# garfieldnate/ray_tracer_challenge

Measured on AMD Instinct MI355X. Metric: Mrays/s, higher is better.
Workload: dtype f32

## Files before the change

ray_tracer_challenge_amd/_lib.py:

```python
import ctypes as C
import os

HERE = os.path.dirname(os.path.abspath(__file__))
LIB_PATH = os.environ.get("RTC_AMD_LIB") or os.path.join(HERE, "librtc_amd.so")

RTC_OK = 0
RTC_ERR_INVALID_ARG, RTC_ERR_UNSUPPORTED, RTC_ERR_NO_LIGHT, RTC_ERR_DEVICE, RTC_ERR_NO_DEVICE = -1, -2, -3, -4, -5
RTC_SPHERE, RTC_PLANE, RTC_CUBE, RTC_CYLINDER, RTC_CONE, RTC_TRIANGLE = 0, 1, 2, 3, 4, 5
(RTC_PATTERN_NONE, RTC_PATTERN_STRIPES, RTC_PATTERN_GRADIENT, RTC_PATTERN_RINGS, RTC_PATTERN_CHECKERS,
 RTC_PATTERN_SINE2D, RTC_PATTERN_TEXTURE_MAP, RTC_PATTERN_CUBE_MAP) = 0, 1, 2, 3, 4, 5, 6, 7
RTC_UV_CHECKERS, RTC_UV_ALIGN_CHECK, RTC_UV_IMAGE = 1, 2, 3
RTC_MAP_SPHERICAL, RTC_MAP_PLANAR, RTC_MAP_CYLINDRICAL = 1, 2, 3
RTC_LIGHT_POINT, RTC_LIGHT_RECT = 0, 1
RTC_JITTER_CONSTANT, RTC_JITTER_HASHED, RTC_JITTER_SEQUENCE = 0, 2, 3
RTC_MAX_DEPTH = 255
RTC_STACK_DEPTH_BASE = 8

FP = C.POINTER(C.c_float)


class rtc_uv_pattern(C.Structure):
    _fields_ = [("kind", C.c_int32), ("width", C.c_float), ("height", C.c_float), ("colors", (C.c_float * 3) * 5),
                ("image_width", C.c_uint32), ("image_height", C.c_uint32), ("image_rgb", C.POINTER(C.c_float))]

# ... 184 lines not shown
         "rtc_diag_refine_block_list": (C.c_uint32, [C.POINTER(C.c_uint32), C.POINTER(C.c_uint32), C.c_uint32, C.c_uint32, C.c_uint32, C.c_double,
                                                     C.c_double, C.c_double, C.POINTER(C.c_uint32), C.c_uint32]),
         "rtc_diag_simulate_dispatch": (C.c_double, [C.POINTER(C.c_uint32), C.c_uint32, C.c_uint32]),
         "rtc_diag_band_walk": (C.c_uint32, [C.c_uint32, C.c_uint32, C.POINTER(rtc_partition), C.POINTER(C.c_uint32), C.c_uint32, C.POINTER(C.c_uint64)]),
         "rtc_diag_scene_tiles": (C.c_uint64, [C.POINTER(C.c_uint8), C.c_uint32, C.c_uint32, C.c_uint32, C.c_uint32, C.POINTER(rtc_partition),
                                               C.POINTER(C.c_uint32), C.POINTER(C.c_uint32), C.c_uint32, C.POINTER(C.c_uint32)]),
         "rtc_diag_rect_launch": (C.c_uint64, [C.c_uint32, C.c_uint32, C.POINTER(rtc_partition), C.POINTER(C.c_uint32), C.c_uint32, C.c_int32,
                                               C.c_uint32, C.POINTER(C.c_uint32)]),
         "rtc_diag_ss_plan": (C.c_uint32, [C.c_uint32, C.c_uint32, C.POINTER(C.c_uint32), C.POINTER(C.c_uint32), C.c_uint32, C.c_uint32, C.c_uint32,
                                           C.c_double, C.POINTER(C.c_uint32), C.c_uint32, C.POINTER(C.c_uint32)]),
         "rtc_diag_ctx_share_log2": (C.c_uint32, [C.c_void_p]),
         "rtc_diag_adaptive_plan": (C.c_uint32, [C.c_uint32, C.c_uint32, C.c_uint32, C.c_uint32, C.c_uint32, C.c_uint64, C.c_uint32,
                                                 C.POINTER(C.c_uint32), C.POINTER(C.c_uint32)]),
         "rtc_diag_ray_keys": (None, [FP, FP, C.c_uint32, FP, C.POINTER(C.c_uint32)]),
         "rtc_diag_reorder_plan": (C.c_uint32, [C.c_uint32, C.c_uint32, C.POINTER(C.c_uint32)]),
         "rtc_diag_scene_plan": (C.c_int, [C.POINTER(rtc_scene), C.POINTER(rtc_camera), C.c_char_p, C.c_uint32, C.POINTER(C.c_uint64)])}

_lib = None
_loaded = {}
DEV_LIB_PATH = os.path.join(HERE, "librtc_amd_dev.so")


class RtcError(RuntimeError):
    def __init__(self, status, message):
        super().__init__("rtc status %d: %s" % (status, message))
        self.status = status


def _preload_torch_hip_runtime():
    import importlib.util
    import sys
# ... 11 lines not shown
            C.CDLL(path, mode=C.RTLD_GLOBAL)
        except OSError:
            pass


def load(path):
    path = os.path.abspath(path)
    if path not in _loaded:
        if not os.path.exists(path):
            raise ImportError(
                "%s is missing: build it with `python -m ray_tracer_challenge_amd.build%s` "
                "(there is no CPU/Python fallback for the render path)" % (path, " --dev" if path.endswith("_dev.so") else ""))
        _preload_torch_hip_runtime()
        L = C.CDLL(path)
        for name, (res, args) in list(SIGNATURES.items()) + list(EXTRA.items()):
            fn = getattr(L, name)
            fn.restype = res
            fn.argtypes = args
        _loaded[path] = L
    return _loaded[path]


def lib():
    global _lib
    if _lib is None:
        _lib = load(LIB_PATH)
    return _lib


class use_library:

# ... 22 lines not shown
```

ray_tracer_challenge_amd/api.py:

```python
import ctypes as C

import numpy as np

from . import _lib as L

f32 = np.float32


def _a(x, n=None):
    arr = np.ascontiguousarray(np.asarray(x, dtype=f32).reshape(-1))
    if n is not None and arr.size != n:
        raise ValueError("expected %d values, got %d" % (n, arr.size))
    return arr


_FLOAT_ARRAYS = {}


def _p(arr):
    n = arr.size
    t = _FLOAT_ARRAYS.get(n)
    if t is None:
        t = _FLOAT_ARRAYS[n] = C.c_float * n
    try:
# ... 690 lines not shown
        self.light = light

    def _c(self):
        return _CScene(self)

    def validate(self, camera=None):
        cs = self._c()
        L.check(L.lib().rtc_scene_validate(C.byref(cs.scene), C.byref(camera._cam) if camera is not None else None))

    def scene_plan(self, camera=None):
        cs = self._c()
        text, digests = C.create_string_buffer(1 << 16), (C.c_uint64 * 4)()
        L.check(L.lib().rtc_diag_scene_plan(C.byref(cs.scene), C.byref(camera._cam) if camera is not None else None, text, len(text), digests))
        return tuple(digests), dict(line.split("=", 1) for line in text.value.decode().splitlines())

    def color_at(self, origins, directions, depth, device=0):
        o = np.ascontiguousarray(np.asarray(origins, dtype=f32).reshape(-1, 4))
        d = np.ascontiguousarray(np.asarray(directions, dtype=f32).reshape(-1, 4))
        out = np.zeros((o.shape[0], 3), dtype=f32)
        cs = self._c()
        L.check(L.lib().rtc_color_at(C.byref(cs.scene), _p(o), _p(d), o.shape[0], int(depth), device, _p(out)))
        return out

    def hit_at(self, origins, directions, light=True, device=0, planes=None):
        o = np.ascontiguousarray(np.asarray(origins, dtype=f32).reshape(-1, 4))
        d = np.ascontiguousarray(np.asarray(directions, dtype=f32).reshape(-1, 4))
        names = list(L.HIT_PLANES) if planes is None else list(planes)
        if not light:
            names = [k for k in names if k != "light"]
        n = o.shape[0]
# ... 190 lines not shown
```

ray_tracer_challenge_amd/csrc/rtc_device.hip:

```cpp
#include <hip/hip_runtime.h>
#include <hip/hiprtc.h>

#include <dlfcn.h>
#include <sys/stat.h>
#include <unistd.h>

#include <cerrno>
#include <chrono>

#include <algorithm>
#include <array>
#include <functional>
#include <queue>
#include <cmath>
#include <cstdio>
#include <cstdlib>
#include <cstring>
#include <fstream>
#include <map>
#include <mutex>
#include <sstream>
#include <string>
#include <utility>
#include <set>
// ... 96 lines not shown
    std::vector<std::string> spec_defs;
    std::string spec_name;
    typedef std::map<int, std::pair<hipFunction_t, std::string>> DeepKernels;
    DeepKernels deep_fn;
    std::string kernel_name;
    int tree_waves = 6;
    bool lazy_jit = false;
    bool jit_deferred = false;
    std::vector<uint8_t> heavy_tiles;
    uint32_t heavy_w = 0, heavy_h = 0;
    std::map<std::array<uint32_t, 5>, BlockList> block_lists;
    float scene_box_coverage = 1.0f;
    uint32_t scene_rect[4] = {0u, 0u, 0u, 0u};
    std::vector<uint8_t> scene_tile_mask;
    uint32_t scene_tiles_w = 0u, scene_tiles_h = 0u;
    struct SceneTileList {
        uint32_t* d = nullptr;
        size_t n = 0;
        unsigned long long traced_pixels = 0ull;
        uint2* d_fill = nullptr;
        size_t n_fill = 0;
    };
    hipStream_t fill_stream = nullptr;
    hipEvent_t ev_fork = nullptr, ev_join = nullptr;
    std::map<std::array<uint32_t, 3>, SceneTileList> scene_tile_lists;
    float scene_rect_coverage = 1.0f;
    std::string kernel_id;
    std::string jit_note;
    std::vector<float4> soa_host;
    std::set<std::pair<const void*, const void*>> warmed;
    std::vector<float> texels_host;
    uint4* d_block_counts = nullptr;
    size_t block_cap = 0;
    void* h_feedback = nullptr;
    size_t h_feedback_cap = 0;
    WfRay* d_wf_rays[4] = {nullptr, nullptr, nullptr, nullptr};
// ... 86 lines not shown
            }
            if (recut) {
                bl.scene_changes = 0u;
                bl.best_ms = bl.loss_ms = 0.0;
                bl.state = timed ? BlockList::TIMED : BlockList::FRESH;
                bl.passes = c->policy.feedback_passes ? c->policy.feedback_passes - 1u : 0u;
            }
        }
        ++it;
    }
}
static void drop_scene_tile_lists(rtc_ctx* c) {
    for (auto& tl : c->scene_tile_lists) {
        if (tl.second.d) (void)hipFree(tl.second.d);
        if (tl.second.d_fill) (void)hipFree(tl.second.d_fill);
    }
    c->scene_tile_lists.clear();
}
static void drop_block_lists(rtc_ctx* c) {
    for (auto& bl : c->block_lists) {
        if (bl.second.d) (void)hipFree(bl.second.d);
        if (bl.second.d_ticks) (void)hipFree(bl.second.d_ticks);
        if (bl.second.ev0) (void)hipEventDestroy(bl.second.ev0);
        if (bl.second.ev1) (void)hipEventDestroy(bl.second.ev1);
    }
    c->block_lists.clear();
}

namespace {

// ... 397 lines not shown
}

static rtc_status order_grid(rtc_ctx* c, BlockList& bl, uint32_t gx, uint32_t gy, uint32_t rows) {
    const Policy& P = c->policy;
    HIP_TRY(hipDeviceSynchronize());
    const size_t nt = bl.n;
    std::vector<uint32_t> launched(nt), ordered;
    void* staging = nullptr;
    HIP_TRY(feedback_staging(c, 4u * nt * sizeof(uint4), &staging));
    uint32_t* ticks = (uint32_t*)staging;
    if (bl.counts) {
        const uint4* counts = (const uint4*)staging;
        HIP_TRY(hipMemcpy(staging, bl.d_ticks, 4u * nt * sizeof(uint4), hipMemcpyDeviceToHost));
        for (size_t i = 0; i < 4u * nt; i++) {
            const uint4 n = counts[i];
            ticks[i] = (n.x - std::min(n.x, n.z)) + 16u * n.y + n.z / 8u;
        }
    } else {
        HIP_TRY(hipMemcpy(staging, bl.d_ticks, 4u * nt * sizeof(uint32_t), hipMemcpyDeviceToHost));
    }
    for (uint32_t by = 0; by < gy; by++)
        for (uint32_t bx = 0; bx < gx; bx++) {
            uint32_t x = bx, y = by;
            if (bl.swizzled) {
                const uint32_t j = (by & 3u) * gx + bx, r = j & 7u;
                y = (by & ~3u) + (r >> 1);
                x = 2u * (j >> 3) + (r & 1u);
            }
            launched[(size_t)by * gx + bx] = tile_word(0u, 16u * x, 16u * y);
        }
    const double wave_slots = 0.85 * 4.0 * compute_units(c) * 6.0;
    bl.state = BlockList::REFINED;
    bl.listed = false;
    {
        std::vector<uint32_t> block_cost(nt), sorted_cost;
        for (size_t b = 0; b < nt; b++) block_cost[b] = std::max(std::max(ticks[4 * b], ticks[4 * b + 1]), std::max(ticks[4 * b + 2], ticks[4 * b + 3]));
        sorted_cost = block_cost;
        std::sort(sorted_cost.begin(), sorted_cost.end(), std::greater<uint32_t>());
        const size_t wg_slots = (size_t)(wave_slots / 4.0);
        const double in_order = simulate_dispatch(block_cost, wg_slots), longest_first = simulate_dispatch(sorted_cost, wg_slots);
        if (P.jit_print) std::fprintf(stderr, "librtc_amd: grid of %zu blocks: modelled frame %.4g in image order, %.4g longest first\n", nt, in_order, longest_first);
        if (!(longest_first < 0.97 * in_order)) return RTC_OK;
    }
    refine_block_list(launched, ticks, c->hdr.width, rows, wave_slots, INFINITY, 0.0, &ordered);
    if (ordered.empty() || ordered.size() > bl.n) return RTC_OK;
    HIP_TRY(grow(&bl.d, &bl.d_cap, ordered.size(), true));
    std::memcpy(staging, ordered.data(), ordered.size() * sizeof(uint32_t));
    HIP_TRY(hipMemcpy(bl.d, staging, ordered.size() * sizeof(uint32_t), hipMemcpyHostToDevice));
    bl.n_listed = ordered.size();
    bl.listed = true;
    return RTC_OK;
}

static hipError_t launch_render(rtc_ctx* c, hipFunction_t spec_fn, dim3 grid, hipStream_t stream, RenderArgs& a) {
    if (c->ss_k != 1u) {
        SsRenderArgs sa;
        sa.fine = a;
// ... 96 lines not shown
    if (!resident) {
        c->soa_host.swap(soa);
        c->texels_host.swap(texels);
    }
    if (same_frame && P.block_feedback) restart_block_lists(c);
    else drop_block_lists(c);
    drop_scene_tile_lists(c);
    c->deep_fn.clear();
    c->simple = plan.simple;
    c->heavy_tiles.swap(plan.heavy_tiles), c->heavy_w = plan.heavy_w, c->heavy_h = plan.heavy_h;
    c->scene_box_coverage = plan.scene_box_coverage;
    std::memcpy(c->scene_rect, plan.scene_rect, sizeof(c->scene_rect));
    c->scene_rect_coverage = plan.scene_rect_coverage;
    c->scene_tile_mask.swap(plan.scene_tile_mask);
    if (!c->scene_tile_mask.empty()) c->scene_tiles_w = plan.scene_tiles_w, c->scene_tiles_h = plan.scene_tiles_h;
    c->spec_shares = plan.spec_shares, c->spec_blocks_y = plan.spec_blocks_y, c->spec_rect = plan.spec_rect;
    if (plan.tree_waves) c->tree_waves = plan.tree_waves;
    c->wf_pays = plan.wf_pays;
    c->wf_disabled = false;
    c->kernel_name = plan.family_name;
    c->spec_defs = plan.spec_defs;
    c->spec_name = plan.spec_name;
    {
        rtc_ctx::Trace& t = c->trace;
        t.defs.clear();
        for (const auto& d : plan.spec_defs)
            t.defs.push_back((d == "-DRTC_SPEC_BLOCKS_Y=1" || d == "-DRTC_SPEC_RECT=1" || d == "-DRTC_SPEC_SHARE=1") ? d.substr(0, d.size() - 1) + "0" : d);
        if (!t.defs.empty()) t.defs.push_back("-DRTC_SPEC_TRACE=1");
        auto renamed = [](const std::string& name) { return name.rfind("render_", 0) == 0 ? "trace_" + name.substr(7) : name; };
        t.family_name = renamed(plan.family_name), t.spec_name = renamed(plan.spec_name);
// ... 158 lines not shown
        c->wf_disabled = true;
        c->events_used--;
        return RTC_OK;
    }
    c->rendered = true;
    c->wf_last = true;
    *used = true;
    return RTC_OK;
}

struct LaunchLists {
    const uint32_t* d_tiles = nullptr;
    uint32_t* d_ticks = nullptr;
    BlockList* timed_list = nullptr;
    void* copy_counts_to = nullptr;
    const rtc_ctx::SceneTileList* scene_tiles = nullptr;
};

static bool scene_recurses(const rtc_ctx* c) {
    const uint32_t stride = padded_count(c->hdr.n_objects);
    for (uint32_t i = 0; i < c->hdr.n_objects; i++) {
        const float4 mb = c->soa_host[soa_index(COL_MAT_B, stride, i)], mc = c->soa_host[soa_index(COL_MAT_C, stride, i)];
        if (!(mb.w == 0.0f) || !(mc.x == 0.0f)) return true;
    }
    return false;
}

static rtc_status block_list_room(rtc_ctx* c) {
    if (c->block_lists.size() >= 256u) {
        HIP_TRY(hipDeviceSynchronize());
        drop_block_lists(c);
// ... 32 lines not shown
        if (bl.state == BlockList::FRESH) {
            bl.state = BlockList::TIMED;
        } else {
            if (bl.ev0 == nullptr) {
                HIP_TRY(hipEventCreate(&bl.ev0));
                HIP_TRY(hipEventCreate(&bl.ev1));
            }
            L->timed_list = &bl;
        }
    }
    L->d_tiles = bl.d;
    lp->run_list(bl.n);
    return RTC_OK;
}

static rtc_status use_scene_tile_list(rtc_ctx* c, const Partition& q, hipStream_t stream, const rtc_ctx::SceneTileList** out) {
    const std::array<uint32_t, 3> key = {q.band_rows, q.n_parts, q.part};
    auto it = c->scene_tile_lists.find(key);
    if (it == c->scene_tile_lists.end()) {
        SceneTilePlan host;
        plan_scene_tiles(TileMask{c->scene_tile_mask.data(), c->scene_tiles_w, c->scene_tiles_h}, c->hdr.width, c->hdr.height, q, &host);
        static_assert(sizeof(FillRun) == sizeof(uint2), "fill_tiles_kernel reads the runs as uint2");
        rtc_ctx::SceneTileList tl;
        tl.n = host.tiles.size();
        tl.n_fill = host.fill.size();
        tl.traced_pixels = host.traced_pixels;
        if (tl.n) {
            HIP_TRY(hipMalloc((void**)&tl.d, tl.n * sizeof(uint32_t)));
            HIP_TRY(hipMemcpyAsync(tl.d, host.tiles.data(), tl.n * sizeof(uint32_t), hipMemcpyHostToDevice, stream));
            if (tl.n_fill) {
                HIP_TRY(hipMalloc((void**)&tl.d_fill, tl.n_fill * sizeof(uint2)));
                HIP_TRY(hipMemcpyAsync(tl.d_fill, host.fill.data(), tl.n_fill * sizeof(uint2), hipMemcpyHostToDevice, stream));
            }
            HIP_TRY(hipStreamSynchronize(stream));
        }
        it = c->scene_tile_lists.emplace(key, tl).first;
    }
    if (it->second.n && !c->fill_stream) {
        HIP_TRY(hipStreamCreateWithFlags(&c->fill_stream, hipStreamNonBlocking));
        HIP_TRY(hipEventCreateWithFlags(&c->ev_fork, hipEventDisableTiming));
        HIP_TRY(hipEventCreateWithFlags(&c->ev_join, hipEventDisableTiming));
    }
    *out = &it->second;
    return RTC_OK;
}

static rtc_status use_grid_feedback(rtc_ctx* c, const Partition& q, uint32_t rows, int32_t depth, bool timed_waves, hipStream_t stream, LaunchPlan* lp,
                                    LaunchLists* L) {
    const std::array<uint32_t, 5> key = {q.band_rows, q.n_parts, q.part, 0xffffffffu, (uint32_t)depth};
    auto it = c->block_lists.find(key);
    if (it == c->block_lists.end()) {
        RTC_TRY(block_list_room(c));
        BlockList bl;
        bl.n = lp->n_workgroups();
        bl.state = BlockList::IDLE;
        it = c->block_lists.emplace(key, bl).first;
    }
    BlockList& bl = it->second;
// ... 61 lines not shown
    a.block_x0 = lp.block_x0, a.block_y0 = lp.block_y0;
    a.fill_wg_rows = lp.fill_wg_rows, a.fill_rows = lp.fill_rows, a.fill_period = lp.fill_period;
    a.fill_x0 = lp.fill_rect[0], a.fill_x1 = lp.fill_rect[1], a.fill_y0 = lp.fill_rect[2], a.fill_y1 = lp.fill_rect[3];
    return a;
}

static bool wavefront_wanted(const rtc_ctx* c, uint32_t rows, int32_t depth) {
    return c->hdr.n_trav != 0u && rows > 0u && depth >= 1 && depth <= RTC_STACK_DEPTH_BASE && (int)depth < (int)WF_MAX_LEVELS && !c->wf_disabled &&
           (size_t)rows * c->hdr.width <= (16u << 20) && c->policy.wavefront == 1 && c->ss_k == 1u;
}

static rtc_status settle_shape(rtc_ctx* c, const Partition& q, uint32_t rows, int32_t depth, uint32_t share_log2, hipFunction_t spec_fn, void* d_out_rgb,
                               bool out_u8, const ProgressPlan* progress, hipStream_t stream, LaunchPlan* lp, LaunchLists* L) {
    const Policy& P = c->policy;
    const bool list_words_fit = c->hdr.width <= 65532u && rows <= 131068u;
    if (lp->shape == LaunchPlan::GRID && share_log2 == 0u && !c->scene_tile_mask.empty() && (q.band_rows & 15u) == 0u && list_words_fit) {
        RTC_TRY(use_scene_tile_list(c, q, stream, &L->scene_tiles));
        if (L->scene_tiles->n) {
            lp->run_scene_tiles(L->scene_tiles->n, c->last_pixels - L->scene_tiles->traced_pixels);
            L->d_tiles = L->scene_tiles->d;
        }
    }
    if (lp->shape == LaunchPlan::GRID && share_log2 == 0u && c->scene_rect[0] < c->scene_rect[1] && c->scene_rect_coverage < P.scene_rect_threshold() &&
        (spec_fn == nullptr || c->spec_rect)) {
        plan_rect_launch(lp, c->hdr.width, c->hdr.height, q, rows, c->last_pixels, c->scene_rect, P.blocks_y == 0 ? 1u : lp->blocks_y, out_u8, P.fill_wgs);
        if (out_u8) HIP_TRY(hipMemsetAsync(d_out_rgb, 0, (size_t)rows * c->hdr.width * 3u, stream));
    }
    if (P.swizzle && lp->plain_grid()) lp->pad_for_swizzle();
    if (lp->plain_grid() && P.block_feedback && P.grid_feedback && progress == nullptr && share_log2 == 0u && list_words_fit &&
        !(c->hdr.n_trav != 0u && P.wavefront))
        RTC_TRY(use_grid_feedback(c, q, rows, depth, spec_fn && c->spec_shares, stream, lp, L));
    if (progress && progress->d_done && lp->plain_grid()) plan_chunks(lp, progress->want_chunks, PROGRESS_MAX_CHUNKS);
// ... 129 lines not shown
        if (n < cap) bands[3 * n] = y0, bands[3 * n + 1] = y1, bands[3 * n + 2] = local0;
        n++;
        for (uint32_t y = y0; y < y1; y++) inverts = inverts && global_row(q, local0 + (y - y0)) == y;
    });
    facts[0] = partition_rows(height, part), facts[1] = traced_pixels(width, height, q), facts[2] = inverts ? 1u : 0u;
    return n;
}
uint64_t rtc_diag_scene_tiles(const uint8_t* mask, uint32_t mask_w, uint32_t mask_h, uint32_t width, uint32_t height, const rtc_partition* part,
                              uint32_t* tiles, uint32_t* fill , uint32_t cap, uint32_t counts[2]) {
    SceneTilePlan plan;
    plan_scene_tiles(TileMask{mask, mask_w, mask_h}, width, height, resolve(part), &plan);
    for (size_t i = 0; i < plan.tiles.size() && i < cap; i++) tiles[i] = plan.tiles[i];
    for (size_t i = 0; i < plan.fill.size() && i < cap; i++) fill[2 * i] = plan.fill[i].x0_n, fill[2 * i + 1] = plan.fill[i].row;
    counts[0] = (uint32_t)plan.tiles.size(), counts[1] = (uint32_t)plan.fill.size();
    return plan.traced_pixels;
}
uint64_t rtc_diag_rect_launch(uint32_t width, uint32_t height, const rtc_partition* part, const uint32_t rect[4], uint32_t blocks_y, int32_t out_u8,
                              uint32_t fill_wgs, uint32_t out[12]) {
    const Partition q = resolve(part);
    LaunchPlan lp;
    plan_rect_launch(&lp, width, height, q, partition_rows(height, part), traced_pixels(width, height, q), rect, blocks_y, out_u8 != 0, fill_wgs);
    const uint32_t v[12] = {lp.grid_x, lp.grid_y, lp.blocks_y, lp.block_x0, lp.block_y0, lp.fill_wg_rows, lp.fill_rows, lp.fill_period,
                            lp.fill_rect[0], lp.fill_rect[1], lp.fill_rect[2], lp.fill_rect[3]};
    std::memcpy(out, v, sizeof(v));
    return lp.extra_rays;
}

uint32_t rtc_diag_ctx_share_log2(rtc_ctx* c) { return c ? c->last_share_log2 : 0u; }
uint32_t rtc_diag_ss_plan(uint32_t k, uint32_t share_log2, const uint32_t* list, const uint32_t* ticks, uint32_t n, uint32_t width, uint32_t rows,
                          double wave_slots, uint32_t* out, uint32_t cap, uint32_t* n_out) {
// ... 1026 lines not shown
```

ray_tracer_challenge_amd/csrc/rtc_launch_plan.h:

```cpp
#ifndef RTC_LAUNCH_PLAN_H
#define RTC_LAUNCH_PLAN_H

#include <algorithm>
#include <cstdint>
#include <cstring>
#include <functional>
#include <queue>
#include <vector>

#include "rtc_internal.h"

namespace rtc {

struct TileMask {
    const uint8_t* bits;
    uint32_t w, h;
};

inline uint32_t tile_word(uint32_t s, uint32_t x0, uint32_t y0) { return (s & 3u) << 30 | (x0 / 4u) << 16 | (s >> 2) << 15 | (y0 / 4u); }
inline uint32_t tile_s(uint32_t t) { return (t >> 30) | ((t >> 13) & 4u); }
inline uint32_t tile_x0(uint32_t t) { return ((t >> 16) & 0x3fffu) << 2; }
inline uint32_t tile_y0(uint32_t t) { return (t & 0x7fffu) << 2; }
inline uint32_t ss_max_share_log2(uint32_t k) { return k == 4u ? 2u : 4u; }
constexpr uint32_t ADAPTIVE_STEP_SLOTS = 64u;
// ... 147 lines not shown
                if (!mask.bits[(size_t)ty * mask.w + tx]) {
                    if (run == 0u) run0 = tx;
                    run++;
                    continue;
                }
                close_run();
                out->tiles.push_back(tile_word(0u, tx * 16u, yl));
                const uint32_t px1 = std::min(width - 1u, tx * 16u + 16u), py1 = std::min(std::min(height - 1u, y1), ty * 16u + 16u);
                if (px1 > tx * 16u && py1 > ty * 16u) out->traced_pixels += (unsigned long long)(px1 - tx * 16u) * (py1 - ty * 16u);
            }
            close_run();
        }
    });
}

struct LaunchPlan {
    enum Shape { GRID, BLOCK_LIST, SCENE_TILES, SCENE_RECT } shape = GRID;
    uint32_t grid_x = 0u, grid_y = 0u;
    uint32_t block_h = 16u;
    uint32_t blocks_y = 1u;
    uint32_t block_x0 = 0u, block_y0 = 0u;
    bool swizzle = false;
    uint32_t fill_wg_rows = 0u, fill_rows = 0u, fill_period = 1u, fill_rect[4] = {0u, 0u, 0u, 0u};
    unsigned long long extra_rays = 0ull;
    uint32_t chunk_block_rows = 1u, n_chunks = 0u;

    bool plain_grid() const { return shape == GRID && blocks_y == 1u; }
    void run_list(size_t n_blocks) { shape = BLOCK_LIST, grid_x = (uint32_t)n_blocks, grid_y = 1u, swizzle = false; }
    void run_scene_tiles(size_t n_tiles, unsigned long long unlaunched) { shape = SCENE_TILES, grid_x = (uint32_t)n_tiles, grid_y = 1u, blocks_y = 1u, extra_rays = unlaunched; }
    void pad_for_swizzle() { swizzle = true, grid_x = (grid_x + 1u) & ~1u, grid_y = (grid_y + 3u) & ~3u; }
// ... 65 lines not shown
```

ray_tracer_challenge_amd/csrc/rtc_oneshot.hip:

```cpp
#include <hip/hip_runtime.h>

#include <algorithm>
#include <chrono>
#include <condition_variable>
#include <cstdio>
#include <cstdlib>
#include <cstring>
#include <functional>
#include <mutex>
#include <thread>
#include <vector>

#include "rtc_internal.h"

using namespace rtc;

#define HIP_TRY(expr)                                                                                \
    do {                                                                                             \
        hipError_t e_ = (expr);                                                                      \
        if (e_ != hipSuccess)                                                                        \
            return fail(RTC_ERR_DEVICE, "%s failed: %s (%s:%d)", #expr, hipGetErrorString(e_), __FILE__, __LINE__); \
    } while (0)
#define RTC_TRY(expr)                  \
    do {                               \
// ... 160 lines not shown
    void* p = nullptr;
    if (hipHostMalloc(&p, bytes ? bytes : 1, hipHostMallocPortable) != hipSuccess) {
        (void)hipGetLastError();
        return nullptr;
    }
    return p;
}
void rtc_host_free(void* p) {
    if (p) (void)hipHostFree(p);
}

void rtc_render_release(void) {
    std::lock_guard<std::mutex> lock(g_mutex);
    for (auto& s : g_state) s.release();
    g_state.clear();
}

rtc_status rtc_render_ex(const rtc_scene* scene, const rtc_camera* camera, int32_t depth, const rtc_opts* opts, void* out,
                         rtc_stats* stats) {
    if (!out || !camera) return fail(RTC_ERR_INVALID_ARG, "rtc_render: null argument");
    if (camera->width == 0 || camera->height == 0) return fail(RTC_ERR_INVALID_ARG, "empty canvas");
    const int32_t dev0 = 0;
    const int32_t* devices = (opts && opts->devices && opts->n_devices) ? opts->devices : &dev0;
    const uint32_t D = (opts && opts->devices && opts->n_devices) ? opts->n_devices : 1u;
    const uint32_t band_rows = (opts && opts->band_rows) ? opts->band_rows : 64u;
    const bool quantize = opts && opts->quantize != 0, on_device = opts && opts->out_on_device != 0;
    int n_visible = 0;
    if (hipGetDeviceCount(&n_visible) != hipSuccess || n_visible <= 0) {
        (void)hipGetLastError();
        return fail(RTC_ERR_NO_DEVICE, "no HIP device visible; librtc_amd has no CPU fallback");
// ... 248 lines not shown
```

ray_tracer_challenge_amd/csrc/rtc_scene_prep.h:

```cpp
#ifndef RTC_SCENE_PREP_H
#define RTC_SCENE_PREP_H

#include <algorithm>
#include <array>
#include <cmath>
#include <cstdint>
#include <cstdio>
#include <cstdlib>
#include <cstring>
#include <string>
#include <utility>
#include <vector>

#include "rtc_internal.h"

namespace rtc {

#define RTC_TRY(expr)                \
    do {                             \
        rtc_status s_ = (expr);      \
        if (s_ != RTC_OK) return s_; \
    } while (0)

inline uint32_t bits_of(float f) {
// ... 166 lines not shown
    if (!(nl > 0.0) || !std::isfinite(nl)) return;
    double big = 0.0;
    for (int a = 0; a < 3; a++) big = std::fmax(big, std::fmax(std::fabs(lo[a]), std::fabs(hi[a])));
    const double pad = pad_scale * (pad_obj / s_min + 1e-5 * (big + d_world));
    if (!std::isfinite(pad)) return;
    rec[0] = make_float4((float)(lo[0] - pad), (float)(lo[1] - pad), (float)(lo[2] - pad), 1.0f);
    rec[1] = make_float4((float)(hi[0] + pad), (float)(hi[1] + pad), (float)(hi[2] + pad), 0.0f);
    rec[2] = make_float4((float)(nrm[0] / nl), (float)(nrm[1] / nl), (float)(nrm[2] / nl), 0.0f);
}

#ifdef RTC_DEV_SWITCHES
#define RTC_DEV_ENV(name) std::getenv(name)
#else
#define RTC_DEV_ENV(name) ((const char*)nullptr)
#endif
struct Policy {
    int specialise = 2;
    bool light_cull = true, dark = true, fast_shadow = true, cell_cull = true, own_blocks = true;
    bool bvh = true, scene_box = true, gates = true, tri_precull = true, block_list = true, quiet = false;
    bool scene_tiles = true;
    bool prune = true;
    int clusters = -1;
    int share_log2 = -1;
    int scene_rect = 1;
    bool swizzle = true;
    bool grid_feedback = true;
    bool block_feedback = true;
    int wavefront = 0;
    std::string jit_cache;
    std::string jit_source, jit_flags;
    bool jit_print = false, cluster_stats = false, tri_naive = false, block_order = true;
    int tree_waves = 0, reg_levels = 0, blocks_y = 0, block_s = -1, block_s_top = -1;
    uint32_t fill_wgs = 0u, tile_fill_wgs = 0u, cluster_min_run = 0u, cluster_leaf = 0u, area_share_waves = 0u, feedback_pct = 85u, feedback_down_pct = 40u, feedback_passes = 2u, feedback_max_s = 4u;
    double cluster_gmax = -1.0;
    int hits_tile = 0;
// ... 1 lines not shown
    static Policy from_env() {
        Policy p;
        auto flag = [](const char* e, bool dflt) { return (e && *e) ? e[0] != '0' : dflt; };
        auto digit = [](const char* e, int lo, int hi, int dflt) { return (e && e[0] >= '0' + lo && e[0] <= '0' + hi && !e[1]) ? e[0] - '0' : dflt; };
        if (const char* e = std::getenv("RTC_AMD_SPECIALIZE")) p.specialise = !*e ? 2 : e[0] == '0' ? 0 : e[0] == '1' ? 1 : 2;
        p.light_cull = flag(std::getenv("RTC_AMD_LIGHT_CULL"), true);
        p.dark = flag(std::getenv("RTC_AMD_DARK"), true);
        p.fast_shadow = flag(std::getenv("RTC_AMD_FAST_SHADOW"), true);
        p.cell_cull = flag(std::getenv("RTC_AMD_CELL_CULL"), true);
        p.own_blocks = flag(std::getenv("RTC_AMD_OWN_BLOCKS"), true);
        p.bvh = flag(std::getenv("RTC_AMD_BVH"), true);
        p.scene_box = flag(std::getenv("RTC_AMD_SCENE_BOX"), true);
        p.gates = flag(std::getenv("RTC_AMD_GATES"), true);
        p.tri_precull = flag(std::getenv("RTC_AMD_TRI_PRECULL"), true);
        p.prune = flag(std::getenv("RTC_AMD_PRUNE"), true);
        p.scene_tiles = flag(std::getenv("RTC_AMD_SCENE_TILES"), true);
        p.block_list = flag(std::getenv("RTC_AMD_BLOCK_LIST"), true);
        p.block_feedback = flag(std::getenv("RTC_AMD_BLOCK_FEEDBACK"), true);
        p.grid_feedback = flag(std::getenv("RTC_AMD_GRID_FEEDBACK"), true);
        p.swizzle = flag(std::getenv("RTC_AMD_SWIZZLE"), true);
        p.quiet = flag(std::getenv("RTC_AMD_QUIET"), false);
        if (const char* e = std::getenv("RTC_AMD_CLUSTERS")) p.clusters = *e ? (e[0] != '0' ? 1 : 0) : -1;
        p.share_log2 = digit(std::getenv("RTC_AMD_SHARE_LOG2"), 0, 3, -1);
        if (const char* e = std::getenv("RTC_AMD_SCENE_RECT")) p.scene_rect = e[0] == '0' ? 0 : e[0] == '2' ? 2 : 1;
        if (const char* e = std::getenv("RTC_AMD_WAVEFRONT")) p.wavefront = (*e && e[0] != '0') ? 1 : 0;
        if (const char* e = std::getenv("RTC_AMD_JIT_CACHE")) p.jit_cache = e;
        if (const char* e = RTC_DEV_ENV("RTC_AMD_JIT_SOURCE")) p.jit_source = e;
        if (const char* e = RTC_DEV_ENV("RTC_AMD_JIT_FLAGS")) p.jit_flags = e;
        p.jit_print = flag(RTC_DEV_ENV("RTC_AMD_JIT_PRINT"), false);
        p.cluster_stats = flag(RTC_DEV_ENV("RTC_AMD_CLUSTER_STATS"), false);
        p.tri_naive = flag(RTC_DEV_ENV("RTC_AMD_TRI_NAIVE"), false);
// ... 967 lines not shown
        const int n = (k + 1) & 3;
        const double gk = g(cx[k], cy[k]), gn = g(cx[n], cy[n]);
        if (gk < 0.0) x0 = std::fmin(x0, cx[k]), x1 = std::fmax(x1, cx[k]), y0 = std::fmin(y0, cy[k]), y1 = std::fmax(y1, cy[k]);
        if ((gk < 0.0) != (gn < 0.0)) {
            const double t = gk / (gk - gn), ex = cx[k] + t * (cx[n] - cx[k]), ey = cy[k] + t * (cy[n] - cy[k]);
            x0 = std::fmin(x0, ex), x1 = std::fmax(x1, ex), y0 = std::fmin(y0, ey), y1 = std::fmax(y1, ey);
        }
    }
    if (!(x0 <= x1) || !(y0 <= y1)) return;
    const long tx0 = std::max(0L, (long)std::floor(x0 / 16.0) - 1), tx1 = std::min((long)tw - 1, (long)std::floor(x1 / 16.0) + 1);
    const long ty0 = std::max(0L, (long)std::floor(y0 / 16.0) - 1), ty1 = std::min((long)th - 1, (long)std::floor(y1 / 16.0) + 1);
    for (long ty = ty0; ty <= ty1; ty++)
        for (long tx = tx0; tx <= tx1; tx++) (*tiles)[(size_t)ty * tw + tx] = 1;
}

struct ScenePlan {
    bool simple = false;
    std::vector<uint8_t> heavy_tiles;
    uint32_t heavy_w = 0u, heavy_h = 0u;
    float scene_box_coverage = 1.0f;
    uint32_t scene_rect[4] = {0u, 0u, 0u, 0u};
    float scene_rect_coverage = 1.0f;
    std::vector<uint8_t> scene_rect_tiles;
    std::vector<uint8_t> scene_tile_mask;
    uint32_t scene_tiles_w = 0u, scene_tiles_h = 0u;
    bool spec_shares = false, spec_blocks_y = false, spec_rect = false;
    int tree_waves = 0;
    bool wf_pays = false;
    std::string family_name;
    std::vector<std::string> spec_defs;
    std::string spec_name;
    bool compile_now = false;
    bool compile_any_size = false, compile_never = false;
};

inline size_t count_tiles(const std::vector<uint8_t>& tiles) {
    size_t n = 0;
    for (uint8_t b : tiles) n += b ? 1u : 0u;
    return n;
}
// ... 17 lines not shown
        project_heavy_boxes(P, box, camera, &covered, &tw, &th);
    }
    if (covered.empty()) covered.assign((size_t)tw * th, 0);
    for (const auto& pl : region.planes) mark_plane_side(pl, camera, &covered, tw, th);
    uint32_t x0 = tw, x1 = 0, y0 = th, y1 = 0;
    for (uint32_t ty = 0; ty < th; ty++)
        for (uint32_t tx = 0; tx < tw; tx++)
            if (covered[(size_t)ty * tw + tx]) x0 = std::min(x0, tx), x1 = std::max(x1, tx + 1u), y0 = std::min(y0, ty), y1 = std::max(y1, ty + 1u);
    if (x0 < x1 && y0 < y1) {
        p->scene_rect[0] = x0, p->scene_rect[1] = x1, p->scene_rect[2] = y0, p->scene_rect[3] = y1;
        p->scene_rect_coverage = (float)((double)(x1 - x0) * (y1 - y0) / ((double)tw * th));
    }
    if (P.jit_print)
        std::fprintf(stderr, "librtc_amd: scene rectangle tiles [%u, %u) x [%u, %u) of %u x %u: %.3f of the frame\n", x0, x1, y0, y1, tw, th,
                     p->scene_rect_coverage);
    if (P.scene_tiles && region.planes.empty() && !region.entry_boxes.empty() && x0 < x1 && y0 < y1) {
        std::vector<uint8_t> each;
        uint32_t ew = 0, eh = 0;
        project_heavy_boxes(P, region.entry_boxes, camera, &each, &ew, &eh);
        const size_t n_each = count_tiles(each);
        if (ew == tw && eh == th && n_each > 0 && 3u * n_each < (size_t)tw * th && 3u * n_each < 2u * (size_t)(x1 - x0) * (y1 - y0)) {
            p->scene_tile_mask = each;
            p->scene_tiles_w = tw, p->scene_tiles_h = th;
        }
        if (P.jit_print) std::fprintf(stderr, "librtc_amd: scene tiles: %zu of %u x %u%s\n", n_each, tw, th, p->scene_tile_mask.empty() ? " (not used)" : "");
    }
    p->scene_rect_tiles.swap(covered);
}

struct MaterialFacts {
    bool any_refl = false, any_refr = false, any_specular = false;
    int reg_levels = 0;
    const char* reg_waves = nullptr;
};
inline MaterialFacts material_facts(const Policy& P, const rtc_scene* scene, uint32_t n) {
    MaterialFacts f;
    for (uint32_t i = 0; i < n; i++) {
        const rtc_material& m = scene->objects[i].material;
        f.any_refl = f.any_refl || !(m.reflective == 0.0f);
        f.any_refr = f.any_refr || !(m.transparency == 0.0f);
// ... 138 lines not shown
```

Before: 2.260 million.

## Extend scene tile lists to plane scenes, swizzle and feedback-order tile lists

Builds scene tile masks for scenes with planes by marking tiles on the visible side of each plane, so tiles that see only background are skipped when enough of the frame is unseen. Scene tile lists are also swizzled into 2x4 tile groups for locality. They can be reordered longest-first using per-wave work counts collected on a timed launch. This adds host syncs, extra count buffers and planning logic, and the plane-side test could mark tiles incorrectly if the margin is wrong.

```diff
diff --git a/ray_tracer_challenge_amd/_lib.py b/ray_tracer_challenge_amd/_lib.py
--- a/ray_tracer_challenge_amd/_lib.py
+++ b/ray_tracer_challenge_amd/_lib.py
@@ -222,7 +222,13 @@
                                                  C.POINTER(C.c_uint32), C.POINTER(C.c_uint32)]),
          "rtc_diag_ray_keys": (None, [FP, FP, C.c_uint32, FP, C.POINTER(C.c_uint32)]),
          "rtc_diag_reorder_plan": (C.c_uint32, [C.c_uint32, C.c_uint32, C.POINTER(C.c_uint32)]),
-         "rtc_diag_scene_plan": (C.c_int, [C.POINTER(rtc_scene), C.POINTER(rtc_camera), C.c_char_p, C.c_uint32, C.POINTER(C.c_uint64)])}
+         "rtc_diag_scene_plan": (C.c_int, [C.POINTER(rtc_scene), C.POINTER(rtc_camera), C.c_char_p, C.c_uint32, C.POINTER(C.c_uint64)]),
+         "rtc_diag_tile_order": (C.c_uint32, [C.POINTER(C.c_uint32), C.POINTER(C.c_uint32), C.c_uint32, C.c_uint32, C.c_uint32, C.POINTER(C.c_uint32), C.c_uint32]),
+         "rtc_diag_wave_work": (C.c_uint32, [C.c_uint32, C.c_uint32, C.c_uint32]),
+         "rtc_diag_longest_first_pays": (C.c_int32, [C.POINTER(C.c_uint32), C.c_uint32, C.c_uint32]),
+         "rtc_diag_scene_tile_mask": (C.c_uint32, [C.POINTER(rtc_scene), C.POINTER(rtc_camera), C.POINTER(C.c_uint8), C.c_uint32, C.POINTER(C.c_uint32)]),
+         "rtc_diag_ctx_scene_tiles": (None, [C.c_void_p, C.POINTER(rtc_partition), C.POINTER(C.c_uint32)]),
+         "rtc_diag_seam_ctx": (C.c_void_p, [C.c_uint32])}
 
 _lib = None
 _loaded = {}
@@ -264,7 +270,13 @@
         _preload_torch_hip_runtime()
         L = C.CDLL(path)
         for name, (res, args) in list(SIGNATURES.items()) + list(EXTRA.items()):
-            fn = getattr(L, name)
+            try:
+                fn = getattr(L, name)
+            except AttributeError:
+                named = os.environ.get("RTC_AMD_LIB")
+                if name.startswith("rtc_diag_") and named and os.path.abspath(named) == path:
+                    continue
+                raise
             fn.restype = res
             fn.argtypes = args
         _loaded[path] = L
diff --git a/ray_tracer_challenge_amd/api.py b/ray_tracer_challenge_amd/api.py
--- a/ray_tracer_challenge_amd/api.py
+++ b/ray_tracer_challenge_amd/api.py
@@ -728,6 +728,16 @@
         L.check(L.lib().rtc_diag_scene_plan(C.byref(cs.scene), C.byref(camera._cam) if camera is not None else None, text, len(text), digests))
         return tuple(digests), dict(line.split("=", 1) for line in text.value.decode().splitlines())
 
+    def scene_tile_mask(self, camera):
+        cs = self._c()
+        tw, th = (camera.width + 15) // 16, (camera.height + 15) // 16
+        mask, dims = np.zeros(tw * th, dtype=np.uint8), (C.c_uint32 * 2)()
+        n = L.lib().rtc_diag_scene_tile_mask(C.byref(cs.scene), C.byref(camera._cam), mask.ctypes.data_as(C.POINTER(C.c_uint8)), mask.size, dims)
+        if n == 0:
+            return None
+        assert (dims[0], dims[1]) == (tw, th) and n == tw * th
+        return mask.reshape(th, tw) != 0
+
     def color_at(self, origins, directions, depth, device=0):
         o = np.ascontiguousarray(np.asarray(origins, dtype=f32).reshape(-1, 4))
         d = np.ascontiguousarray(np.asarray(directions, dtype=f32).reshape(-1, 4))
diff --git a/ray_tracer_challenge_amd/csrc/rtc_device.hip b/ray_tracer_challenge_amd/csrc/rtc_device.hip
--- a/ray_tracer_challenge_amd/csrc/rtc_device.hip
+++ b/ray_tracer_challenge_amd/csrc/rtc_device.hip
@@ -134,12 +134,17 @@
     uint32_t scene_rect[4] = {0u, 0u, 0u, 0u};
     std::vector<uint8_t> scene_tile_mask;
     uint32_t scene_tiles_w = 0u, scene_tiles_h = 0u;
+    bool scene_tiles_sparse = false;
     struct SceneTileList {
         uint32_t* d = nullptr;
         size_t n = 0;
         unsigned long long traced_pixels = 0ull;
         uint2* d_fill = nullptr;
         size_t n_fill = 0;
+        std::vector<uint32_t> host;
+        uint4* d_counts = nullptr;
+        enum { IDLE, FRESH, TIMED, SETTLED } state = IDLE;
+        bool ordered = false;
     };
     hipStream_t fill_stream = nullptr;
     hipEvent_t ev_fork = nullptr, ev_join = nullptr;
@@ -256,6 +261,7 @@
     for (auto& tl : c->scene_tile_lists) {
         if (tl.second.d) (void)hipFree(tl.second.d);
         if (tl.second.d_fill) (void)hipFree(tl.second.d_fill);
+        if (tl.second.d_counts) (void)hipFree(tl.second.d_counts);
     }
     c->scene_tile_lists.clear();
 }
@@ -683,7 +689,7 @@
         HIP_TRY(hipMemcpy(staging, bl.d_ticks, 4u * nt * sizeof(uint4), hipMemcpyDeviceToHost));
         for (size_t i = 0; i < 4u * nt; i++) {
             const uint4 n = counts[i];
-            ticks[i] = (n.x - std::min(n.x, n.z)) + 16u * n.y + n.z / 8u;
+            ticks[i] = wave_work(n.x, n.y, n.z);
         }
     } else {
         HIP_TRY(hipMemcpy(staging, bl.d_ticks, 4u * nt * sizeof(uint32_t), hipMemcpyDeviceToHost));
@@ -702,14 +708,10 @@
     bl.state = BlockList::REFINED;
     bl.listed = false;
     {
-        std::vector<uint32_t> block_cost(nt), sorted_cost;
-        for (size_t b = 0; b < nt; b++) block_cost[b] = std::max(std::max(ticks[4 * b], ticks[4 * b + 1]), std::max(ticks[4 * b + 2], ticks[4 * b + 3]));
-        sorted_cost = block_cost;
-        std::sort(sorted_cost.begin(), sorted_cost.end(), std::greater<uint32_t>());
-        const size_t wg_slots = (size_t)(wave_slots / 4.0);
-        const double in_order = simulate_dispatch(block_cost, wg_slots), longest_first = simulate_dispatch(sorted_cost, wg_slots);
+        double in_order = 0.0, longest_first = 0.0;
+        const bool pays = longest_first_pays(ticks, nt, (size_t)(wave_slots / 4.0), &in_order, &longest_first);
         if (P.jit_print) std::fprintf(stderr, "librtc_amd: grid of %zu blocks: modelled frame %.4g in image order, %.4g longest first\n", nt, in_order, longest_first);
-        if (!(longest_first < 0.97 * in_order)) return RTC_OK;
+        if (!pays) return RTC_OK;
     }
     refine_block_list(launched, ticks, c->hdr.width, rows, wave_slots, INFINITY, 0.0, &ordered);
     if (ordered.empty() || ordered.size() > bl.n) return RTC_OK;
@@ -836,6 +838,7 @@
     c->scene_rect_coverage = plan.scene_rect_coverage;
     c->scene_tile_mask.swap(plan.scene_tile_mask);
     if (!c->scene_tile_mask.empty()) c->scene_tiles_w = plan.scene_tiles_w, c->scene_tiles_h = plan.scene_tiles_h;
+    c->scene_tiles_sparse = plan.scene_tiles_sparse;
     c->spec_shares = plan.spec_shares, c->spec_blocks_y = plan.spec_blocks_y, c->spec_rect = plan.spec_rect;
     if (plan.tree_waves) c->tree_waves = plan.tree_waves;
     c->wf_pays = plan.wf_pays;
@@ -1024,7 +1027,7 @@
     uint32_t* d_ticks = nullptr;
     BlockList* timed_list = nullptr;
     void* copy_counts_to = nullptr;
-    const rtc_ctx::SceneTileList* scene_tiles = nullptr;
+    rtc_ctx::SceneTileList* scene_tiles = nullptr;
 };
 
 static bool scene_recurses(const rtc_ctx* c) {
@@ -1087,12 +1090,48 @@
     return RTC_OK;
 }
 
-static rtc_status use_scene_tile_list(rtc_ctx* c, const Partition& q, hipStream_t stream, const rtc_ctx::SceneTileList** out) {
+static rtc_status order_scene_tiles(rtc_ctx* c, rtc_ctx::SceneTileList& tl, uint32_t rows) {
+    HIP_TRY(hipDeviceSynchronize());
+    tl.state = rtc_ctx::SceneTileList::SETTLED;
+    void* staging = nullptr;
+    HIP_TRY(feedback_staging(c, 4u * tl.n * sizeof(uint4), &staging));
+    HIP_TRY(hipMemcpy(staging, tl.d_counts, 4u * tl.n * sizeof(uint4), hipMemcpyDeviceToHost));
+    const uint4* counts = (const uint4*)staging;
+    uint32_t* ticks = (uint32_t*)staging;
+    for (size_t i = 0; i < 4u * tl.n; i++) {
+        const uint4 n = counts[i];
+        ticks[i] = wave_work(n.x, n.y, n.z);
+    }
+    double in_order = 0.0, longest_first = 0.0;
+    const bool pays = longest_first_pays(ticks, tl.n, (size_t)(0.85 * compute_units(c) * 6.0), &in_order, &longest_first);
+    if (c->policy.jit_print)
+        std::fprintf(stderr, "librtc_amd: scene tiles: list of %zu: modelled frame %.4g in list order, %.4g longest first\n", tl.n, in_order, longest_first);
+    if (!pays) return RTC_OK;
+    std::vector<uint32_t> ordered;
+    order_tile_list(tl.host, ticks, c->hdr.width, rows, &ordered);
+    if (ordered.size() != tl.n) return RTC_OK;
+    HIP_TRY(hipMemcpy(tl.d, ordered.data(), tl.n * sizeof(uint32_t), hipMemcpyHostToDevice));
+    tl.host.swap(ordered);
+    tl.ordered = true;
+    return RTC_OK;
+}
+
+static rtc_status use_scene_tile_list(rtc_ctx* c, const Partition& q, uint32_t rows, bool feedback, hipStream_t stream, LaunchLists* L) {
+    const Policy& P = c->policy;
     const std::array<uint32_t, 3> key = {q.band_rows, q.n_parts, q.part};
     auto it = c->scene_tile_lists.find(key);
     if (it == c->scene_tile_lists.end()) {
+        if (c->scene_tile_lists.size() >= 256u) {
+            HIP_TRY(hipDeviceSynchronize());
+            drop_scene_tile_lists(c);
+        }
         SceneTilePlan host;
         plan_scene_tiles(TileMask{c->scene_tile_mask.data(), c->scene_tiles_w, c->scene_tiles_h}, c->hdr.width, c->hdr.height, q, &host);
+        if (P.swizzle) {
+            std::vector<uint32_t> permuted;
+            swizzle_tile_list(host.tiles, c->hdr.width, rows, &permuted);
+            host.tiles.swap(permuted);
+        }
         static_assert(sizeof(FillRun) == sizeof(uint2), "fill_tiles_kernel reads the runs as uint2");
         rtc_ctx::SceneTileList tl;
         tl.n = host.tiles.size();
@@ -1107,14 +1146,26 @@
             }
             HIP_TRY(hipStreamSynchronize(stream));
         }
+        tl.host.swap(host.tiles);
         it = c->scene_tile_lists.emplace(key, tl).first;
+    }
+    rtc_ctx::SceneTileList& tl = it->second;
+    if (tl.n && feedback) {
+        if (tl.state == rtc_ctx::SceneTileList::TIMED) RTC_TRY(order_scene_tiles(c, tl, rows));
+        if (tl.state == rtc_ctx::SceneTileList::IDLE) {
+            tl.state = rtc_ctx::SceneTileList::FRESH;
+        } else if (tl.state == rtc_ctx::SceneTileList::FRESH) {
+            if (!tl.d_counts) HIP_TRY(hipMalloc((void**)&tl.d_counts, 4u * tl.n * sizeof(uint4)));
+            L->copy_counts_to = tl.d_counts;
+            tl.state = rtc_ctx::SceneTileList::TIMED;
+        }
     }
     if (it->second.n && !c->fill_stream) {
         HIP_TRY(hipStreamCreateWithFlags(&c->fill_stream, hipStreamNonBlocking));
         HIP_TRY(hipEventCreateWithFlags(&c->ev_fork, hipEventDisableTiming));
         HIP_TRY(hipEventCreateWithFlags(&c->ev_join, hipEventDisableTiming));
     }
-    *out = &it->second;
+    L->scene_tiles = &it->second;
     return RTC_OK;
 }
 
@@ -1206,8 +1257,9 @@
                                bool out_u8, const ProgressPlan* progress, hipStream_t stream, LaunchPlan* lp, LaunchLists* L) {
     const Policy& P = c->policy;
     const bool list_words_fit = c->hdr.width <= 65532u && rows <= 131068u;
-    if (lp->shape == LaunchPlan::GRID && share_log2 == 0u && !c->scene_tile_mask.empty() && (q.band_rows & 15u) == 0u && list_words_fit) {
-        RTC_TRY(use_scene_tile_list(c, q, stream, &L->scene_tiles));
+    if (lp->shape == LaunchPlan::GRID && share_log2 == 0u && !c->scene_tile_mask.empty() && (q.band_rows & 15u) == 0u && list_words_fit &&
+        (progress == nullptr || c->scene_tiles_sparse)) {
+        RTC_TRY(use_scene_tile_list(c, q, rows, P.block_feedback && P.grid_feedback && progress == nullptr, stream, L));
         if (L->scene_tiles->n) {
             lp->run_scene_tiles(L->scene_tiles->n, c->last_pixels - L->scene_tiles->traced_pixels);
             L->d_tiles = L->scene_tiles->d;
@@ -1367,6 +1419,41 @@
     for (size_t i = 0; i < plan.fill.size() && i < cap; i++) fill[2 * i] = plan.fill[i].x0_n, fill[2 * i + 1] = plan.fill[i].row;
     counts[0] = (uint32_t)plan.tiles.size(), counts[1] = (uint32_t)plan.fill.size();
     return plan.traced_pixels;
+}
+uint32_t rtc_diag_tile_order(const uint32_t* list, const uint32_t* ticks, uint32_t n, uint32_t width, uint32_t rows, uint32_t* out, uint32_t cap) {
+    std::vector<uint32_t> l(list, list + n), made;
+    if (ticks) order_tile_list(l, ticks, width, rows, &made);
+    else swizzle_tile_list(l, width, rows, &made);
+    for (size_t i = 0; i < made.size() && i < cap; i++) out[i] = made[i];
+    return (uint32_t)made.size();
+}
+uint32_t rtc_diag_wave_work(uint32_t rays, uint32_t shade_points, uint32_t culled) { return wave_work(rays, shade_points, culled); }
+int32_t rtc_diag_longest_first_pays(const uint32_t* ticks, uint32_t n_blocks, uint32_t wg_slots) { return longest_first_pays(ticks, n_blocks, wg_slots) ? 1 : 0; }
+uint32_t rtc_diag_scene_tile_mask(const rtc_scene* scene, const rtc_camera* camera, uint8_t* mask, uint32_t cap, uint32_t dims[2]) {
+    dims[0] = dims[1] = 0u;
+    if (!scene || !camera) return 0u;
+    const Policy P = Policy::from_env();
+    SceneHdr hdr;
+    std::vector<float4> soa;
+    std::vector<float> texels, heavy_boxes;
+    SceneRegion region;
+    if (flatten(P, scene, camera, &hdr, &soa, &texels, &heavy_boxes, &region) != RTC_OK) return 0u;
+    ScenePlan p;
+    plan_coverage(P, hdr, camera, region, &p);
+    if (p.scene_tile_mask.empty() || p.scene_tile_mask.size() > cap) return 0u;
+    std::memcpy(mask, p.scene_tile_mask.data(), p.scene_tile_mask.size());
+    dims[0] = p.scene_tiles_w, dims[1] = p.scene_tiles_h;
+    return (uint32_t)p.scene_tile_mask.size();
+}
+void rtc_diag_ctx_scene_tiles(rtc_ctx* c, const rtc_partition* part, uint32_t out[3]) {
+    out[0] = out[1] = out[2] = 0u;
+    if (!c) return;
+    const Partition q = resolve(part);
+    auto it = c->scene_tile_lists.find({q.band_rows, q.n_parts, q.part});
+    if (it == c->scene_tile_lists.end()) return;
+    const rtc_ctx::SceneTileList& tl = it->second;
+    out[0] = (uint32_t)tl.n, out[1] = (uint32_t)tl.n_fill;
+    out[2] = tl.state <= rtc_ctx::SceneTileList::FRESH ? 0u : tl.state == rtc_ctx::SceneTileList::TIMED ? 1u : tl.ordered ? 3u : 2u;
 }
 uint64_t rtc_diag_rect_launch(uint32_t width, uint32_t height, const rtc_partition* part, const uint32_t rect[4], uint32_t blocks_y, int32_t out_u8,
                               uint32_t fill_wgs, uint32_t out[12]) {
diff --git a/ray_tracer_challenge_amd/csrc/rtc_launch_plan.h b/ray_tracer_challenge_amd/csrc/rtc_launch_plan.h
--- a/ray_tracer_challenge_amd/csrc/rtc_launch_plan.h
+++ b/ray_tracer_challenge_amd/csrc/rtc_launch_plan.h
@@ -2,6 +2,7 @@
 #define RTC_LAUNCH_PLAN_H
 
 #include <algorithm>
+#include <cmath>
 #include <cstdint>
 #include <cstring>
 #include <functional>
@@ -185,6 +186,37 @@
     });
 }
 
+inline uint32_t wave_work(uint32_t rays, uint32_t shade_points, uint32_t culled) { return (rays - std::min(rays, culled)) + 16u * shade_points + culled / 8u; }
+inline bool longest_first_pays(const uint32_t* ticks, size_t n_blocks, size_t wg_slots, double* in_order = nullptr, double* longest_first = nullptr) {
+    std::vector<uint32_t> block_cost(n_blocks), sorted_cost;
+    for (size_t b = 0; b < n_blocks; b++) block_cost[b] = std::max(std::max(ticks[4 * b], ticks[4 * b + 1]), std::max(ticks[4 * b + 2], ticks[4 * b + 3]));
+    sorted_cost = block_cost;
+    std::sort(sorted_cost.begin(), sorted_cost.end(), std::greater<uint32_t>());
+    const double a = simulate_dispatch(block_cost, wg_slots), b = simulate_dispatch(sorted_cost, wg_slots);
+    if (in_order) *in_order = a;
+    if (longest_first) *longest_first = b;
+    return b < 0.97 * a;
+}
+inline void swizzle_tile_list(const std::vector<uint32_t>& list, uint32_t width, uint32_t rows, std::vector<uint32_t>* out) {
+    const uint32_t tw = (width + 15u) / 16u, th = (rows + 15u) / 16u, gx = (tw + 1u) & ~1u;
+    std::vector<int32_t> index((size_t)tw * th, -1);
+    out->clear();
+    for (size_t i = 0; i < list.size(); i++) {
+        const uint32_t tx = tile_x0(list[i]) / 16u, ty = tile_y0(list[i]) / 16u;
+        if (tx >= tw || ty >= th || index[(size_t)ty * tw + tx] >= 0) return (void)(*out = list);
+        index[(size_t)ty * tw + tx] = (int32_t)i;
+    }
+    out->reserve(list.size());
+    for (uint32_t ty0 = 0; ty0 < th; ty0 += 4u)
+        for (uint32_t j = 0; j < 4u * gx; j++) {
+            const uint32_t tx = 2u * (j >> 3) + (j & 1u), ty = ty0 + ((j & 7u) >> 1);
+            if (tx < tw && ty < th && index[(size_t)ty * tw + tx] >= 0) out->push_back(list[(size_t)index[(size_t)ty * tw + tx]]);
+        }
+}
+inline void order_tile_list(const std::vector<uint32_t>& list, const uint32_t* ticks, uint32_t width, uint32_t rows, std::vector<uint32_t>* out) {
+    refine_block_list(list, ticks, width, rows, 1.0, INFINITY, 0.0, out);
+}
+
 struct LaunchPlan {
     enum Shape { GRID, BLOCK_LIST, SCENE_TILES, SCENE_RECT } shape = GRID;
     uint32_t grid_x = 0u, grid_y = 0u;
diff --git a/ray_tracer_challenge_amd/csrc/rtc_oneshot.hip b/ray_tracer_challenge_amd/csrc/rtc_oneshot.hip
--- a/ray_tracer_challenge_amd/csrc/rtc_oneshot.hip
+++ b/ray_tracer_challenge_amd/csrc/rtc_oneshot.hip
@@ -198,6 +198,11 @@
     std::lock_guard<std::mutex> lock(g_mutex);
     for (auto& s : g_state) s.release();
     g_state.clear();
+}
+
+rtc_ctx* rtc_diag_seam_ctx(uint32_t k) {
+    std::lock_guard<std::mutex> lock(g_mutex);
+    return k < g_state.size() ? g_state[k].ctx : nullptr;
 }
 
 rtc_status rtc_render_ex(const rtc_scene* scene, const rtc_camera* camera, int32_t depth, const rtc_opts* opts, void* out,
diff --git a/ray_tracer_challenge_amd/csrc/rtc_scene_prep.h b/ray_tracer_challenge_amd/csrc/rtc_scene_prep.h
--- a/ray_tracer_challenge_amd/csrc/rtc_scene_prep.h
+++ b/ray_tracer_challenge_amd/csrc/rtc_scene_prep.h
@@ -204,11 +204,12 @@
 #else
 #define RTC_DEV_ENV(name) ((const char*)nullptr)
 #endif
+constexpr uint32_t SCENE_TILES_UNSEEN_PCT = 20u;
 struct Policy {
     int specialise = 2;
     bool light_cull = true, dark = true, fast_shadow = true, cell_cull = true, own_blocks = true;
     bool bvh = true, scene_box = true, gates = true, tri_precull = true, block_list = true, quiet = false;
-    bool scene_tiles = true;
+    int scene_tiles = 1;
     bool prune = true;
     int clusters = -1;
     int share_log2 = -1;
@@ -240,7 +241,7 @@
         p.gates = flag(std::getenv("RTC_AMD_GATES"), true);
         p.tri_precull = flag(std::getenv("RTC_AMD_TRI_PRECULL"), true);
         p.prune = flag(std::getenv("RTC_AMD_PRUNE"), true);
-        p.scene_tiles = flag(std::getenv("RTC_AMD_SCENE_TILES"), true);
+        if (const char* e = std::getenv("RTC_AMD_SCENE_TILES")) p.scene_tiles = e[0] == '0' ? 0 : e[0] == '2' ? 2 : 1;
         p.block_list = flag(std::getenv("RTC_AMD_BLOCK_LIST"), true);
         p.block_feedback = flag(std::getenv("RTC_AMD_BLOCK_FEEDBACK"), true);
         p.grid_feedback = flag(std::getenv("RTC_AMD_GRID_FEEDBACK"), true);
@@ -1238,6 +1239,26 @@
         for (long tx = tx0; tx <= tx1; tx++) (*tiles)[(size_t)ty * tw + tx] = 1;
 }
 
+inline void mark_plane_tiles(const std::array<double, 4>& row, const rtc_camera* cam, std::vector<uint8_t>* tiles, uint32_t tw, uint32_t th) {
+    const float* m = cam->inv;
+    const double y_o = row[0] * m[3] + row[1] * m[7] + row[2] * m[11] + row[3];
+    double col[3];
+    for (int k = 0; k < 3; k++) col[k] = row[0] * m[k] + row[1] * m[4 + k] + row[2] * m[8 + k];
+    const double sz = cam->pixel_size, a = -col[0] * sz, b = -col[1] * sz;
+    const double c0 = col[0] * (cam->half_width - 0.5 * sz) + col[1] * (cam->half_height - 0.5 * sz) - col[2];
+    if (!std::isfinite(y_o) || !std::isfinite(a) || !std::isfinite(b) || !std::isfinite(c0) || y_o == 0.0) {
+        std::fill(tiles->begin(), tiles->end(), (uint8_t)1);
+        return;
+    }
+    const double sgn = y_o > 0.0 ? 1.0 : -1.0, margin = 8.0 * (std::fabs(a) + std::fabs(b));
+    auto g = [&](double px, double py) { return sgn * (a * px + b * py + c0) - margin; };
+    for (uint32_t ty = 0; ty < th; ty++)
+        for (uint32_t tx = 0; tx < tw; tx++) {
+            const double x0 = 16.0 * tx, y0 = 16.0 * ty;
+            if (g(x0, y0) < 0.0 || g(x0 + 16.0, y0) < 0.0 || g(x0, y0 + 16.0) < 0.0 || g(x0 + 16.0, y0 + 16.0) < 0.0) (*tiles)[(size_t)ty * tw + tx] = 1;
+        }
+}
+
 struct ScenePlan {
     bool simple = false;
     std::vector<uint8_t> heavy_tiles;
@@ -1248,6 +1269,7 @@
     std::vector<uint8_t> scene_rect_tiles;
     std::vector<uint8_t> scene_tile_mask;
     uint32_t scene_tiles_w = 0u, scene_tiles_h = 0u;
+    bool scene_tiles_sparse = false;
     bool spec_shares = false, spec_blocks_y = false, spec_rect = false;
     int tree_waves = 0;
     bool wf_pays = false;
@@ -1295,16 +1317,24 @@
     if (P.jit_print)
         std::fprintf(stderr, "librtc_amd: scene rectangle tiles [%u, %u) x [%u, %u) of %u x %u: %.3f of the frame\n", x0, x1, y0, y1, tw, th,
                      p->scene_rect_coverage);
-    if (P.scene_tiles && region.planes.empty() && !region.entry_boxes.empty() && x0 < x1 && y0 < y1) {
+    if (P.scene_tiles != 0 && (!region.entry_boxes.empty() || !region.planes.empty()) && x0 < x1 && y0 < y1) {
         std::vector<uint8_t> each;
-        uint32_t ew = 0, eh = 0;
-        project_heavy_boxes(P, region.entry_boxes, camera, &each, &ew, &eh);
-        const size_t n_each = count_tiles(each);
-        if (ew == tw && eh == th && n_each > 0 && 3u * n_each < (size_t)tw * th && 3u * n_each < 2u * (size_t)(x1 - x0) * (y1 - y0)) {
-            p->scene_tile_mask = each;
-            p->scene_tiles_w = tw, p->scene_tiles_h = th;
-        }
-        if (P.jit_print) std::fprintf(stderr, "librtc_amd: scene tiles: %zu of %u x %u%s\n", n_each, tw, th, p->scene_tile_mask.empty() ? " (not used)" : "");
+        uint32_t ew = tw, eh = th;
+        if (!region.entry_boxes.empty()) project_heavy_boxes(P, region.entry_boxes, camera, &each, &ew, &eh);
+        else each.assign((size_t)tw * th, 0);
+        if (ew == tw && eh == th && each.size() == (size_t)tw * th) {
+            for (uint8_t& b : each) b = b ? 1 : 0;
+            for (const auto& pl : region.planes) mark_plane_tiles(pl, camera, &each, tw, th);
+            const size_t n_each = count_tiles(each), n_all = (size_t)tw * th, unseen = n_all - n_each;
+            const bool sparse = region.planes.empty() && 3u * n_each < n_all && 3u * n_each < 2u * (size_t)(x1 - x0) * (y1 - y0);
+            const bool wanted = P.scene_tiles == 2 || (region.planes.empty() ? sparse : 100u * unseen >= (size_t)SCENE_TILES_UNSEEN_PCT * n_all);
+            if (n_each > 0 && unseen > 0 && wanted) {
+                p->scene_tile_mask = each;
+                p->scene_tiles_w = tw, p->scene_tiles_h = th;
+                p->scene_tiles_sparse = sparse;
+            }
+            if (P.jit_print) std::fprintf(stderr, "librtc_amd: scene tiles: %zu of %u x %u%s\n", n_each, tw, th, p->scene_tile_mask.empty() ? " (not used)" : "");
+        }
     }
     p->scene_rect_tiles.swap(covered);
 }
```

Result: faster. 2.378 million (median of 6 runs) (+5.2%).
